# A-Nasiri-M/sap3d_tensorflow

Hardware: AMD Instinct MI355X
Metric: clips/s (16x112x112 fwd+bwd) (higher is better)
Workload: dtype f32

## Files before the change

### sap3d_tensorflow_amd/csrc/head.hip

```cpp
#include "p3d_kernels.h"
#include "det_reduce.h"

namespace {

__device__ __forceinline__ float4 ld4(const float* p) { return *reinterpret_cast<const float4*>(p); }

__global__ __launch_bounds__(256) void head_fwd_kernel(HeadArgs a) {
    P3D_CHAIN_PRIO();
    extern __shared__ float kw[];
    const int C = a.C;
    for (int i = threadIdx.x; i < 27 * C; i += blockDim.x) kw[i] = a.k[i];
    __syncthreads();
    const long long total = (long long)a.N * a.D * a.H * a.W;
    const float bias = a.bias[0];
    for (long long g = (long long)blockIdx.x * blockDim.x + threadIdx.x; g < total; g += (long long)gridDim.x * blockDim.x) {
        long long t = g;
        const int w = (int)(t % a.W); t /= a.W;
        const int h = (int)(t % a.H); t /= a.H;
        const int d = (int)(t % a.D); const int n = (int)(t / a.D);
        float out[8];
#pragma unroll
        for (int q = 0; q < 8; ++q) out[q] = bias;
        for (int dd = 0; dd < 2; ++dd) {
            if (d - dd < 0) continue;
            for (int dh = 0; dh < 2; ++dh) {
                if (h - dh < 0) continue;
                for (int dw = 0; dw < 2; ++dw) {
                    if (w - dw < 0) continue;
                    const float* xr = a.x + ((((long long)n * a.D + (d - dd)) * a.H + (h - dh)) * a.W + (w - dw)) * C;
                    const int nkd = dd ? 1 : 2, nkh = dh ? 1 : 2, nkw = dw ? 1 : 2;
                    for (int c = 0; c < C; c += 4) {
                        const float4 xv = ld4(xr + c);
                        for (int a0 = 0; a0 < nkd; ++a0) {
                            const int kd = dd ? 2 : a0, pd = dd ? 0 : a0;
                            for (int a1 = 0; a1 < nkh; ++a1) {
                                const int kh = dh ? 2 : a1, ph = dh ? 0 : a1;
                                for (int a2 = 0; a2 < nkw; ++a2) {
                                    const int kk = dw ? 2 : a2, pw = dw ? 0 : a2;
                                    const float* kp = kw + ((kd * 3 + kh) * 3 + kk) * C + c;
                                    out[(pd * 2 + ph) * 2 + pw] += xv.x * kp[0] + xv.y * kp[1] + xv.z * kp[2] + xv.w * kp[3];
                                }
                            }
                        }
                    }
                }
            }
        }
        const int Do = 2 * a.D, Ho = 2 * a.H, Wo = 2 * a.W;
#pragma unroll
        for (int pd = 0; pd < 2; ++pd)
#pragma unroll
            for (int ph = 0; ph < 2; ++ph) {
                const long long o = (((long long)n * Do + 2 * d + pd) * Ho + 2 * h + ph) * Wo + 2 * w;
                const float v0 = out[(pd * 2 + ph) * 2], v1 = out[(pd * 2 + ph) * 2 + 1];
                *reinterpret_cast<float2*>(a.logits + o) = make_float2(v0, v1);
                *reinterpret_cast<float2*>(a.pred + o) =
                    a.sigmoid ? make_float2(1.f / (1.f + expf(-v0)), 1.f / (1.f + expf(-v1))) : make_float2(v0, v1);
            }
    }
}

template <int L>
__global__ __launch_bounds__(256) void head_fwd_lanes_kernel(HeadArgs a) {
    P3D_CHAIN_PRIO();
    extern __shared__ float kw[];
    const int C = a.C;
    for (int i = threadIdx.x; i < 27 * C; i += blockDim.x) kw[i] = a.k[i];
    __syncthreads();
    const long long total = (long long)a.N * a.D * a.H * a.W;
    const float bias = a.bias[0];
    const int part = threadIdx.x % L, c = part * 4;
    const long long stride = (long long)gridDim.x * (256 / L);
    for (long long g = (long long)blockIdx.x * (256 / L) + threadIdx.x / L; g < total; g += stride) {
        long long t = g;
        const int w = (int)(t % a.W); t /= a.W;
        const int h = (int)(t % a.H); t /= a.H;
        const int d = (int)(t % a.D); const int n = (int)(t / a.D);
        float out[8];
#pragma unroll
        for (int q = 0; q < 8; ++q) out[q] = 0.f;
#pragma unroll
        for (int dd = 0; dd < 2; ++dd)
#pragma unroll
            for (int dh = 0; dh < 2; ++dh)
#pragma unroll
                for (int dw = 0; dw < 2; ++dw) {
                    if (d - dd < 0 || h - dh < 0 || w - dw < 0) continue;
                    const float4 xv = ld4(a.x + ((((long long)n * a.D + (d - dd)) * a.H + (h - dh)) * a.W + (w - dw)) * C + c);
#pragma unroll
                    for (int a0 = 0; a0 < (dd ? 1 : 2); ++a0)
#pragma unroll
                        for (int a1 = 0; a1 < (dh ? 1 : 2); ++a1)
#pragma unroll
                            for (int a2 = 0; a2 < (dw ? 1 : 2); ++a2) {
                                const int kd = dd ? 2 : a0, pd = dd ? 0 : a0, kh = dh ? 2 : a1, ph = dh ? 0 : a1, kk = dw ? 2 : a2, pw = dw ? 0 : a2;
                                const float4 kv = *reinterpret_cast<const float4*>(kw + ((kd * 3 + kh) * 3 + kk) * C + c);
                                out[(pd * 2 + ph) * 2 + pw] += xv.x * kv.x + xv.y * kv.y + xv.z * kv.z + xv.w * kv.w;
                            }
                }
#pragma unroll
        for (int o = L / 2; o > 0; o >>= 1)
#pragma unroll
            for (int q = 0; q < 8; ++q) out[q] += __shfl_xor(out[q], o);
        if (part == 0) {
            const int Do = 2 * a.D, Ho = 2 * a.H, Wo = 2 * a.W;
#pragma unroll
            for (int pd = 0; pd < 2; ++pd)
#pragma unroll
                for (int ph = 0; ph < 2; ++ph) {
                    const long long o = (((long long)n * Do + 2 * d + pd) * Ho + 2 * h + ph) * Wo + 2 * w;
                    const float v0 = out[(pd * 2 + ph) * 2] + bias, v1 = out[(pd * 2 + ph) * 2 + 1] + bias;
                    *reinterpret_cast<float2*>(a.logits + o) = make_float2(v0, v1);
                    *reinterpret_cast<float2*>(a.pred + o) =
                        a.sigmoid ? make_float2(1.f / (1.f + expf(-v0)), 1.f / (1.f + expf(-v1))) : make_float2(v0, v1);
                }
        }
    }
}

__global__ __launch_bounds__(256) void head_bwd_input_kernel(HeadArgs a) {
    P3D_CHAIN_PRIO();
    extern __shared__ float kw[];
    const int C = a.C, c4n = C >> 2;
    for (int i = threadIdx.x; i < 27 * C; i += blockDim.x) kw[i] = a.k[i];
    __syncthreads();
    const long long total = (long long)a.N * a.D * a.H * a.W * c4n;
    const int Do = 2 * a.D, Ho = 2 * a.H, Wo = 2 * a.W;
    for (long long i = (long long)blockIdx.x * blockDim.x + threadIdx.x; i < total; i += (long long)gridDim.x * blockDim.x) {
        long long t = i / c4n;
        const int c = (int)(i - t * c4n) << 2;
        const long long g = t;
        const int w = (int)(t % a.W); t /= a.W;
        const int h = (int)(t % a.H); t /= a.H;
        const int d = (int)(t % a.D); const int n = (int)(t / a.D);
        float4 acc = make_float4(0.f, 0.f, 0.f, 0.f);
        for (int kd = 0; kd < 3; ++kd) {
            const int od = 2 * d + kd;
            if (od >= Do) continue;
            for (int kh = 0; kh < 3; ++kh) {
                const int oh = 2 * h + kh;
                if (oh >= Ho) continue;
                for (int kk = 0; kk < 3; ++kk) {
                    const int ow = 2 * w + kk;
                    if (ow >= Wo) continue;
                    const float gdl = a.dlogits[(((long long)n * Do + od) * Ho + oh) * Wo + ow];
                    const float* kp = kw + ((kd * 3 + kh) * 3 + kk) * C + c;
                    acc.x += gdl * kp[0]; acc.y += gdl * kp[1]; acc.z += gdl * kp[2]; acc.w += gdl * kp[3];
                }
            }
        }
        *reinterpret_cast<float4*>(a.dx + g * C + c) = acc;
    }
}

__global__ __launch_bounds__(256) void head_bwd_filter_kernel(HeadArgs a) {
    __shared__ float red[256];
    const int C = a.C;
    const int lanes = 256 / C;
    const int c = threadIdx.x % C, sub = threadIdx.x / C;
    const long long total = (long long)a.N * a.D * a.H * a.W;
    const int Do = 2 * a.D, Ho = 2 * a.H, Wo = 2 * a.W;
    float acc[27];
#pragma unroll
    for (int q = 0; q < 27; ++q) acc[q] = 0.f;
    float bsum = 0.f;
    if (sub < lanes) {
        for (long long g = (long long)blockIdx.x * lanes + sub; g < total; g += (long long)gridDim.x * lanes) {
            long long t = g;
            const int w = (int)(t % a.W); t /= a.W;
            const int h = (int)(t % a.H); t /= a.H;
            const int d = (int)(t % a.D); const int n = (int)(t / a.D);
            const float xv = a.x[g * C + c];
#pragma unroll
            for (int kd = 0; kd < 3; ++kd)
#pragma unroll
                for (int kh = 0; kh < 3; ++kh)
#pragma unroll
                    for (int kk = 0; kk < 3; ++kk) {
                        const int od = 2 * d + kd, oh = 2 * h + kh, ow = 2 * w + kk;
                        float gdl = 0.f;
                        if (od < Do && oh < Ho && ow < Wo) gdl = a.dlogits[(((long long)n * Do + od) * Ho + oh) * Wo + ow];
                        acc[(kd * 3 + kh) * 3 + kk] += gdl * xv;
                        if (c == 0 && kd < 2 && kh < 2 && kk < 2) bsum += gdl;
                    }
        }
    }
    for (int q = 0; q < 27; ++q) {
        red[threadIdx.x] = (sub < lanes) ? acc[q] : 0.f;
        __syncthreads();
        if (threadIdx.x < C) {
            float s = 0.f;
            for (int l = 0; l < lanes; ++l) s += red[l * C + threadIdx.x];
            p3d_store_wt(a.part, ((size_t)blockIdx.x * 28 + q) * C + threadIdx.x, s);
        }
        __syncthreads();
    }
    red[threadIdx.x] = (sub < lanes && c == 0) ? bsum : 0.f;
    __syncthreads();
    if (threadIdx.x == 0) {
        float s = 0.f;
        for (int l = 0; l < lanes; ++l) s += red[l * C];
        p3d_store_wt(a.part, ((size_t)blockIdx.x * 28 + 27) * C, s);
    }
    __shared__ int last_flag;
    if (!p3d_last_block_wt(a.counter, gridDim.x, &last_flag)) return;
    for (int i = threadIdx.x; i < 27 * C + 1; i += blockDim.x) {
        const size_t slot = i < 27 * C ? (size_t)i : (size_t)27 * C;
        float t = 0.f;
#pragma unroll 8
        for (unsigned b = 0; b < gridDim.x; ++b) t += a.part[(size_t)b * 28 * C + slot];
        if (i < 27 * C) a.dk[i] += t; else a.dbias[0] += t;
    }
}

constexpr int HEAD_FOLD = 32;
__global__ __launch_bounds__(256) void head_bwd_filter4_kernel(HeadArgs a) {
    __shared__ float4 red[256];
    __shared__ int last_flag;
    const int C = a.C, L = C >> 2, R = 256 / L;
    const int lane = threadIdx.x % L, rs = threadIdx.x / L;
    const bool live = rs < R;
    const long long total = (long long)a.N * a.D * a.H * a.W;
    const int Do = 2 * a.D, Ho = 2 * a.H, Wo = 2 * a.W;
    float4 acc[27];
#pragma unroll
    for (int q = 0; q < 27; ++q) acc[q] = make_float4(0.f, 0.f, 0.f, 0.f);
    float bsum = 0.f;
    if (live) {
        for (long long g = (long long)blockIdx.x * R + rs; g < total; g += (long long)gridDim.x * R) {
            long long t = g;
            const int w = (int)(t % a.W); t /= a.W;
            const int h = (int)(t % a.H); t /= a.H;
            const int d = (int)(t % a.D); const int n = (int)(t / a.D);
            const float4 xv = *reinterpret_cast<const float4*>(a.x + g * C + lane * 4);
#pragma unroll
            for (int kd = 0; kd < 3; ++kd)
#pragma unroll
                for (int kh = 0; kh < 3; ++kh)
#pragma unroll
                    for (int kk = 0; kk < 3; ++kk) {
                        const int od = 2 * d + kd, oh = 2 * h + kh, ow = 2 * w + kk;
                        float gdl = 0.f;
                        if (od < Do && oh < Ho && ow < Wo) gdl = a.dlogits[(((long long)n * Do + od) * Ho + oh) * Wo + ow];
                        float4& s = acc[(kd * 3 + kh) * 3 + kk];
                        s.x = fmaf(gdl, xv.x, s.x); s.y = fmaf(gdl, xv.y, s.y); s.z = fmaf(gdl, xv.z, s.z); s.w = fmaf(gdl, xv.w, s.w);
                        if (lane == 0 && kd < 2 && kh < 2 && kk < 2) bsum += gdl;
                    }
        }
    }
#pragma unroll
    for (int q = 0; q < 27; ++q) {
        red[threadIdx.x] = live ? acc[q] : make_float4(0.f, 0.f, 0.f, 0.f);
        __syncthreads();
        if (threadIdx.x < L) {
            float4 s = red[threadIdx.x];
            for (int r = 1; r < R; ++r) { const float4 v = red[r * L + threadIdx.x]; s.x += v.x; s.y += v.y; s.z += v.z; s.w += v.w; }
            p3d_store_wt4(a.part, (size_t)blockIdx.x * 28 * C + q * C + threadIdx.x * 4, s);
        }
        __syncthreads();
    }
    red[threadIdx.x].x = (live && lane == 0) ? bsum : 0.f;
    __syncthreads();
    if (threadIdx.x == 0) {
        float s = 0.f;
        for (int r = 0; r < R; ++r) s += red[r * L].x;
        p3d_store_wt(a.part, (size_t)blockIdx.x * 28 * C + 27 * C, s);
    }
    const int nvals = 27 * C + 1;
    const unsigned ngroups = (gridDim.x + HEAD_FOLD - 1) / HEAD_FOLD, group = blockIdx.x / HEAD_FOLD;
    const unsigned first = group * HEAD_FOLD, in_group = min((unsigned)HEAD_FOLD, gridDim.x - first);
    float* gpart = a.part + (size_t)gridDim.x * 28 * C;
    if (!p3d_last_block_wt(a.counter + 1 + group, in_group, &last_flag)) return;
    for (int i = threadIdx.x; i < nvals; i += blockDim.x) {
        float t = 0.f;
#pragma unroll 8
        for (unsigned b = 0; b < in_group; ++b) t += a.part[(size_t)(first + b) * 28 * C + i];
        p3d_store_wt(gpart, (size_t)group * 28 * C + i, t);
    }
    if (!p3d_last_block_wt(a.counter, ngroups, &last_flag)) return;
    for (int i = threadIdx.x; i < nvals; i += blockDim.x) {
        float t = 0.f;
#pragma unroll 8
        for (unsigned gidx = 0; gidx < ngroups; ++gidx) t += gpart[(size_t)gidx * 28 * C + i];
        if (i < 27 * C) a.dk[i] += t; else a.dbias[0] += t;
    }
}

__global__ __launch_bounds__(256) void headc_fwd_kernel(HeadArgs a) {
    P3D_CHAIN_PRIO();
    extern __shared__ float kw[];
    const int C = a.C;
    for (int i = threadIdx.x; i < 27 * C; i += blockDim.x) kw[i] = a.k[i];
    __syncthreads();
    const long long total = (long long)a.N * a.D * a.H * a.W;
    const float bias = a.bias[0];
    for (long long g = (long long)blockIdx.x * blockDim.x + threadIdx.x; g < total; g += (long long)gridDim.x * blockDim.x) {
        long long t = g;
        const int w = (int)(t % a.W); t /= a.W;
        const int h = (int)(t % a.H); t /= a.H;
        const int d = (int)(t % a.D); const int n = (int)(t / a.D);
        float out = bias;
        for (int kd = 0; kd < 3; ++kd) {
            const int id = d + kd - 1;
            if (id < 0 || id >= a.D) continue;
            for (int kh = 0; kh < 3; ++kh) {
                const int ih = h + kh - 1;
                if (ih < 0 || ih >= a.H) continue;
                for (int kk = 0; kk < 3; ++kk) {
                    const int iw = w + kk - 1;
                    if (iw < 0 || iw >= a.W) continue;
                    const float* xr = a.x + ((((long long)n * a.D + id) * a.H + ih) * a.W + iw) * C;
                    const float* kp = kw + ((kd * 3 + kh) * 3 + kk) * C;
                    for (int c = 0; c < C; c += 4) {
                        const float4 xv = ld4(xr + c);
                        out += xv.x * kp[c] + xv.y * kp[c + 1] + xv.z * kp[c + 2] + xv.w * kp[c + 3];
                    }
                }
            }
        }
        a.logits[g] = out;
        a.pred[g] = a.sigmoid ? 1.f / (1.f + expf(-out)) : out;
    }
}

__global__ __launch_bounds__(256) void headc_bwd_input_kernel(HeadArgs a) {
    P3D_CHAIN_PRIO();
    extern __shared__ float kw[];
    const int C = a.C, c4n = C >> 2;
    for (int i = threadIdx.x; i < 27 * C; i += blockDim.x) kw[i] = a.k[i];
    __syncthreads();
    const long long total = (long long)a.N * a.D * a.H * a.W * c4n;
    for (long long i = (long long)blockIdx.x * blockDim.x + threadIdx.x; i < total; i += (long long)gridDim.x * blockDim.x) {
        long long t = i / c4n;
        const int c = (int)(i - t * c4n) << 2;
        const long long g = t;
        const int w = (int)(t % a.W); t /= a.W;
        const int h = (int)(t % a.H); t /= a.H;
        const int d = (int)(t % a.D); const int n = (int)(t / a.D);
        float4 acc = make_float4(0.f, 0.f, 0.f, 0.f);
        for (int kd = 0; kd < 3; ++kd) {
            const int od = d - kd + 1;
            if (od < 0 || od >= a.D) continue;
            for (int kh = 0; kh < 3; ++kh) {
                const int oh = h - kh + 1;
                if (oh < 0 || oh >= a.H) continue;
                for (int kk = 0; kk < 3; ++kk) {
                    const int ow = w - kk + 1;
                    if (ow < 0 || ow >= a.W) continue;
                    const float gdl = a.dlogits[(((long long)n * a.D + od) * a.H + oh) * a.W + ow];
                    const float* kp = kw + ((kd * 3 + kh) * 3 + kk) * C + c;
                    acc.x += gdl * kp[0]; acc.y += gdl * kp[1]; acc.z += gdl * kp[2]; acc.w += gdl * kp[3];
                }
            }
        }
        *reinterpret_cast<float4*>(a.dx + g * C + c) = acc;
    }
}

__global__ __launch_bounds__(256) void headc_bwd_filter_kernel(HeadArgs a) {
    __shared__ float red[256];
    const int C = a.C;
    const int lanes = 256 / C;
    const int c = threadIdx.x % C, sub = threadIdx.x / C;
    const long long total = (long long)a.N * a.D * a.H * a.W;
    float acc[27];
#pragma unroll
    for (int q = 0; q < 27; ++q) acc[q] = 0.f;
    float bsum = 0.f;
    if (sub < lanes) {
        for (long long g = (long long)blockIdx.x * lanes + sub; g < total; g += (long long)gridDim.x * lanes) {
            long long t = g;
            const int w = (int)(t % a.W); t /= a.W;
            const int h = (int)(t % a.H); t /= a.H;
            const int d = (int)(t % a.D); const int n = (int)(t / a.D);
            const float xv = a.x[g * C + c];
            if (c == 0) bsum += a.dlogits[g];
#pragma unroll
            for (int kd = 0; kd < 3; ++kd)
#pragma unroll
                for (int kh = 0; kh < 3; ++kh)
#pragma unroll
                    for (int kk = 0; kk < 3; ++kk) {
                        const int od = d - kd + 1, oh = h - kh + 1, ow = w - kk + 1;
                        float gdl = 0.f;
                        if (od >= 0 && od < a.D && oh >= 0 && oh < a.H && ow >= 0 && ow < a.W)
                            gdl = a.dlogits[(((long long)n * a.D + od) * a.H + oh) * a.W + ow];
                        acc[(kd * 3 + kh) * 3 + kk] += gdl * xv;
                    }
        }
    }
    for (int q = 0; q < 27; ++q) {
        red[threadIdx.x] = (sub < lanes) ? acc[q] : 0.f;
        __syncthreads();
        if (threadIdx.x < C) {
            float s = 0.f;
            for (int l = 0; l < lanes; ++l) s += red[l * C + threadIdx.x];
            p3d_store_wt(a.part, ((size_t)blockIdx.x * 28 + q) * C + threadIdx.x, s);
        }
        __syncthreads();
    }
    red[threadIdx.x] = (sub < lanes && c == 0) ? bsum : 0.f;
    __syncthreads();
    if (threadIdx.x == 0) {
        float s = 0.f;
        for (int l = 0; l < lanes; ++l) s += red[l * C];
        p3d_store_wt(a.part, ((size_t)blockIdx.x * 28 + 27) * C, s);
    }
    __shared__ int last_flag;
    if (!p3d_last_block_wt(a.counter, gridDim.x, &last_flag)) return;
    for (int i = threadIdx.x; i < 27 * C + 1; i += blockDim.x) {
        const size_t slot = i < 27 * C ? (size_t)i : (size_t)27 * C;
        float t = 0.f;
#pragma unroll 8
        for (unsigned b = 0; b < gridDim.x; ++b) t += a.part[(size_t)b * 28 * C + slot];
        if (i < 27 * C) a.dk[i] += t; else a.dbias[0] += t;
    }
}

}

hipError_t p3d_headc_fwd(const HeadArgs& a, hipStream_t s, HeadLaunch* done) {
    if ((a.C & 3) || a.C < 4 || a.C > 256) return hipErrorInvalidValue;
    const long long total = (long long)a.N * a.D * a.H * a.W;
    long long b = (total + 255) / 256;
    if (b > 8192) b = 8192;
    hipLaunchKernelGGL(headc_fwd_kernel, dim3((unsigned)b), dim3(256), 27 * a.C * sizeof(float), s, a);
    if (done) { done->kernel = P3D_HEAD_STRIDE1; done->blocks = (unsigned)b; }
    return hipGetLastError();
}

hipError_t p3d_headc_bwd_input(const HeadArgs& a, hipStream_t s) {
    if ((a.C & 3) || a.C < 4 || a.C > 256) return hipErrorInvalidValue;
    const long long total = (long long)a.N * a.D * a.H * a.W * (a.C >> 2);
    long long b = (total + 255) / 256;
    if (b > 8192) b = 8192;
    hipLaunchKernelGGL(headc_bwd_input_kernel, dim3((unsigned)b), dim3(256), 27 * a.C * sizeof(float), s, a);
    return hipGetLastError();
}

hipError_t p3d_headc_bwd_filter(const HeadArgs& a, hipStream_t s, HeadLaunch* done) {
    if (a.C > 256 || a.C < 1) return hipErrorInvalidValue;
    const long long total = (long long)a.N * a.D * a.H * a.W;
    const int lanes = 256 / a.C;
    long long b = (total + (long long)lanes * 32 - 1) / ((long long)lanes * 32);
    if (b > 256) b = 256;
    if (b < 1) b = 1;
    HeadArgs aa = a;
    const hipError_t e = p3d_stream_scratch(s, (size_t)b * 28 * a.C, 1, &aa.part, &aa.counter);
    if (e != hipSuccess) return e;
    hipLaunchKernelGGL(headc_bwd_filter_kernel, dim3((unsigned)b), dim3(256), 0, s, aa);
    if (done) { done->kernel = P3D_HEAD_STRIDE1; done->blocks = (unsigned)b; }
    return hipGetLastError();
}

hipError_t p3d_head_fwd(const HeadArgs& a, hipStream_t s, int path, HeadLaunch* done) {
    if ((a.C & 3) || a.C < 4 || a.C > 256) return hipErrorInvalidValue;
    if (path != P3D_HEAD_RULE && path != P3D_HEAD_LANES && path != P3D_HEAD_GENERIC) return hipErrorInvalidValue;
    const long long total = (long long)a.N * a.D * a.H * a.W;
    const int L = a.C >> 2;
    const bool lanes_ok = L > 1 && L <= 64 && (L & (L - 1)) == 0 && (reinterpret_cast<uintptr_t>(a.x) & 15) == 0;
    if (path == P3D_HEAD_LANES && !lanes_ok) return hipErrorInvalidValue;
    if (path == P3D_HEAD_LANES || (path == P3D_HEAD_RULE && lanes_ok)) {
        long long b = (total * L + 255) / 256;
        if (b > 16384) b = 16384;
        const size_t sm = 27 * a.C * sizeof(float);
#define P3D_HL(L_) case L_: hipLaunchKernelGGL(head_fwd_lanes_kernel<L_>, dim3((unsigned)b), dim3(256), sm, s, a); break;
        switch (L) { P3D_HL(2) P3D_HL(4) P3D_HL(8) P3D_HL(16) P3D_HL(32) P3D_HL(64) }
#undef P3D_HL
        if (done) { done->kernel = P3D_HEAD_LANES; done->blocks = (unsigned)b; }
        return hipGetLastError();
    }
    long long b = (total + 255) / 256;
    if (b > 8192) b = 8192;
    hipLaunchKernelGGL(head_fwd_kernel, dim3((unsigned)b), dim3(256), 27 * a.C * sizeof(float), s, a);
    if (done) { done->kernel = P3D_HEAD_GENERIC; done->blocks = (unsigned)b; }
    return hipGetLastError();
}

hipError_t p3d_head_bwd_input(const HeadArgs& a, hipStream_t s) {
    if ((a.C & 3) || a.C < 4 || a.C > 256) return hipErrorInvalidValue;
    const long long total = (long long)a.N * a.D * a.H * a.W * (a.C >> 2);
    long long b = (total + 255) / 256;
    if (b > 8192) b = 8192;
    hipLaunchKernelGGL(head_bwd_input_kernel, dim3((unsigned)b), dim3(256), 27 * a.C * sizeof(float), s, a);
    return hipGetLastError();
}

hipError_t p3d_head_bwd_filter(const HeadArgs& a, hipStream_t s, int path, HeadLaunch* done) {
    if (a.C > 256 || a.C < 1) return hipErrorInvalidValue;
    if (path != P3D_HEAD_RULE && path != P3D_HEAD_FILTER4 && path != P3D_HEAD_FILTER1) return hipErrorInvalidValue;
    const long long total = (long long)a.N * a.D * a.H * a.W;
    const bool four_ok = (a.C & 3) == 0 && (reinterpret_cast<uintptr_t>(a.x) & 15) == 0;
    if (path == P3D_HEAD_FILTER4 && !four_ok) return hipErrorInvalidValue;
    if (path == P3D_HEAD_FILTER4 || (path == P3D_HEAD_RULE && four_ok)) {
        const int R = 256 / (a.C >> 2);
        long long b = (total + (long long)R * 4 - 1) / ((long long)R * 4);
        if (b > 1024) b = 1024;
        if (b < 1) b = 1;
        const long long groups = (b + HEAD_FOLD - 1) / HEAD_FOLD;
        HeadArgs aa = a;
        const hipError_t e = p3d_stream_scratch(s, (size_t)(b + groups) * 28 * a.C, (int)(1 + groups), &aa.part, &aa.counter);
        if (e != hipSuccess) return e;
        hipLaunchKernelGGL(head_bwd_filter4_kernel, dim3((unsigned)b), dim3(256), 0, s, aa);
        if (done) { done->kernel = P3D_HEAD_FILTER4; done->blocks = (unsigned)b; }
        return hipGetLastError();
    }
    const int lanes = 256 / a.C;
    long long b = (total + (long long)lanes * 32 - 1) / ((long long)lanes * 32);
    if (b > 256) b = 256;
    if (b < 1) b = 1;
    HeadArgs aa = a;
    const hipError_t e = p3d_stream_scratch(s, (size_t)b * 28 * a.C, 1, &aa.part, &aa.counter);
    if (e != hipSuccess) return e;
    hipLaunchKernelGGL(head_bwd_filter_kernel, dim3((unsigned)b), dim3(256), 0, s, aa);
    if (done) { done->kernel = P3D_HEAD_FILTER1; done->blocks = (unsigned)b; }
    return hipGetLastError();
}
```

Measured before the change: 527.0.

## Keep head taps in registers, use DPP reductions and 32-bit indexing

For lane counts up to 16, the forward head kernel now loads its 27 filter taps per channel group into registers instead of staging them in shared memory. It issues all eight input loads up front, reduces across lanes with DPP row shifts, and caps the grid at a resident-sized launch. The input-gradient kernel is rebuilt the same way: one thread group per voxel, register-held taps, branch-free clamped loads, and 32-bit index math when the volume is small enough. The filter-gradient block reduction moves to wave-level DPP/shuffle sums followed by one cross-wave shared pass, replacing 27 barrier pairs. The cost is higher register pressure under a launch bound of 3 blocks per CU, and the DPP lane-above adds must line up correctly with the lane layout.

```diff
diff --git a/sap3d_tensorflow_amd/csrc/head.hip b/sap3d_tensorflow_amd/csrc/head.hip
--- a/sap3d_tensorflow_amd/csrc/head.hip
+++ b/sap3d_tensorflow_amd/csrc/head.hip
@@ -60,9 +60,108 @@
     }
 }
 
+__device__ __forceinline__ void head_position(const HeadArgs& a, long long g, bool narrow, int& n, int& d, int& h, int& w) {
+    if (narrow) {
+        unsigned t = (unsigned)g;
+        w = (int)(t % (unsigned)a.W); t /= (unsigned)a.W;
+        h = (int)(t % (unsigned)a.H); t /= (unsigned)a.H;
+        d = (int)(t % (unsigned)a.D); n = (int)(t / (unsigned)a.D);
+    } else {
+        long long t = g;
+        w = (int)(t % a.W); t /= a.W;
+        h = (int)(t % a.H); t /= a.H;
+        d = (int)(t % a.D); n = (int)(t / a.D);
+    }
+}
+
+template <int O>
+__device__ __forceinline__ float add_from_lane_above(float v) {
+    const int up = __builtin_amdgcn_update_dpp(0, __float_as_int(v), 0x100 + O, 0xf, 0xf, true);
+    return v + __int_as_float(up);
+}
+
+__device__ __forceinline__ void head_taps(const HeadArgs& a, int c, float4 (&kv)[27]) {
+#pragma unroll
+    for (int q = 0; q < 27; ++q) {
+        const float* kp = a.k + q * a.C + c;
+        kv[q] = make_float4(kp[0], kp[1], kp[2], kp[3]);
+    }
+}
+
 template <int L>
-__global__ __launch_bounds__(256) void head_fwd_lanes_kernel(HeadArgs a) {
-    P3D_CHAIN_PRIO();
+__device__ __forceinline__ void head_fwd_lanes_resident(const HeadArgs& a) {
+    const int C = a.C;
+    const long long total = (long long)a.N * a.D * a.H * a.W;
+    const bool narrow = total < (1ll << 31);
+    const float bias = a.bias[0];
+    const int part = threadIdx.x % L, c = part * 4;
+    float4 kv[27];
+    head_taps(a, c, kv);
+    const long long stride = (long long)gridDim.x * (256 / L);
+    for (long long g = (long long)blockIdx.x * (256 / L) + threadIdx.x / L; g < total; g += stride) {
+        int n, d, h, w;
+        head_position(a, g, narrow, n, d, h, w);
+        float4 xs[8];
+#pragma unroll
+        for (int dd = 0; dd < 2; ++dd)
+#pragma unroll
+            for (int dh = 0; dh < 2; ++dh)
+#pragma unroll
+                for (int dw = 0; dw < 2; ++dw) {
+                    const bool in = d - dd >= 0 && h - dh >= 0 && w - dw >= 0;
+                    const int id = max(d - dd, 0), ih = max(h - dh, 0), iw = max(w - dw, 0);
+                    const float4 xv = ld4(a.x + ((((long long)n * a.D + id) * a.H + ih) * a.W + iw) * C + c);
+                    xs[(dd * 2 + dh) * 2 + dw] = in ? xv : make_float4(0.f, 0.f, 0.f, 0.f);
+                }
+        float out[8];
+#pragma unroll
+        for (int q = 0; q < 8; ++q) out[q] = 0.f;
+#pragma unroll
+        for (int dd = 0; dd < 2; ++dd)
+#pragma unroll
+            for (int dh = 0; dh < 2; ++dh)
+#pragma unroll
+                for (int dw = 0; dw < 2; ++dw) {
+                    const float4 xv = xs[(dd * 2 + dh) * 2 + dw];
+#pragma unroll
+                    for (int a0 = 0; a0 < (dd ? 1 : 2); ++a0)
+#pragma unroll
+                        for (int a1 = 0; a1 < (dh ? 1 : 2); ++a1)
+#pragma unroll
+                            for (int a2 = 0; a2 < (dw ? 1 : 2); ++a2) {
+                                const int kd = dd ? 2 : a0, pd = dd ? 0 : a0, kh = dh ? 2 : a1, ph = dh ? 0 : a1, kk = dw ? 2 : a2, pw = dw ? 0 : a2;
+                                const float4 k4 = kv[(kd * 3 + kh) * 3 + kk];
+                                out[(pd * 2 + ph) * 2 + pw] += xv.x * k4.x + xv.y * k4.y + xv.z * k4.z + xv.w * k4.w;
+                            }
+                }
+#pragma unroll
+        for (int q = 0; q < 8; ++q) {
+            float v = out[q];
+            if (L > 32) v += __shfl_xor(v, 32);
+            if (L > 16) v += __shfl_xor(v, 16);
+            if (L > 8) v = add_from_lane_above<8>(v);
+            if (L > 4) v = add_from_lane_above<4>(v);
+            if (L > 2) v = add_from_lane_above<2>(v);
+            out[q] = add_from_lane_above<1>(v);
+        }
+        if (part == 0) {
+            const int Do = 2 * a.D, Ho = 2 * a.H, Wo = 2 * a.W;
+#pragma unroll
+            for (int pd = 0; pd < 2; ++pd)
+#pragma unroll
+                for (int ph = 0; ph < 2; ++ph) {
+                    const long long o = (((long long)n * Do + 2 * d + pd) * Ho + 2 * h + ph) * Wo + 2 * w;
+                    const float v0 = out[(pd * 2 + ph) * 2] + bias, v1 = out[(pd * 2 + ph) * 2 + 1] + bias;
+                    *reinterpret_cast<float2*>(a.logits + o) = make_float2(v0, v1);
+                    *reinterpret_cast<float2*>(a.pred + o) =
+                        a.sigmoid ? make_float2(1.f / (1.f + expf(-v0)), 1.f / (1.f + expf(-v1))) : make_float2(v0, v1);
+                }
+        }
+    }
+}
+
+template <int L>
+__device__ __forceinline__ void head_fwd_lanes_staged(const HeadArgs& a) {
     extern __shared__ float kw[];
     const int C = a.C;
     for (int i = threadIdx.x; i < 27 * C; i += blockDim.x) kw[i] = a.k[i];
@@ -118,36 +217,41 @@
     }
 }
 
-__global__ __launch_bounds__(256) void head_bwd_input_kernel(HeadArgs a) {
+template <int L>
+__global__ __launch_bounds__(256, 3) void head_fwd_lanes_kernel(HeadArgs a) {
     P3D_CHAIN_PRIO();
-    extern __shared__ float kw[];
-    const int C = a.C, c4n = C >> 2;
-    for (int i = threadIdx.x; i < 27 * C; i += blockDim.x) kw[i] = a.k[i];
-    __syncthreads();
-    const long long total = (long long)a.N * a.D * a.H * a.W * c4n;
+    if constexpr (L <= 16) head_fwd_lanes_resident<L>(a); else head_fwd_lanes_staged<L>(a);
+}
+
+__global__ __launch_bounds__(256, 3) void head_bwd_input_kernel(HeadArgs a) {
+    P3D_CHAIN_PRIO();
+    const int C = a.C, L = C >> 2, R = 256 / L;
+    const int part = threadIdx.x % L, rs = threadIdx.x / L, c = part * 4;
+    if (rs >= R) return;
+    const long long total = (long long)a.N * a.D * a.H * a.W;
+    const bool narrow = total < (1ll << 31);
     const int Do = 2 * a.D, Ho = 2 * a.H, Wo = 2 * a.W;
-    for (long long i = (long long)blockIdx.x * blockDim.x + threadIdx.x; i < total; i += (long long)gridDim.x * blockDim.x) {
-        long long t = i / c4n;
-        const int c = (int)(i - t * c4n) << 2;
-        const long long g = t;
-        const int w = (int)(t % a.W); t /= a.W;
-        const int h = (int)(t % a.H); t /= a.H;
-        const int d = (int)(t % a.D); const int n = (int)(t / a.D);
+    float4 kv[27];
+    head_taps(a, c, kv);
+    for (long long g = (long long)blockIdx.x * R + rs; g < total; g += (long long)gridDim.x * R) {
+        int n, d, h, w;
+        head_position(a, g, narrow, n, d, h, w);
+        float gdl[27];
+#pragma unroll
+        for (int kd = 0; kd < 3; ++kd)
+#pragma unroll
+            for (int kh = 0; kh < 3; ++kh)
+#pragma unroll
+                for (int kk = 0; kk < 3; ++kk) {
+                    const int od = 2 * d + kd, oh = 2 * h + kh, ow = 2 * w + kk;
+                    const bool in = od < Do && oh < Ho && ow < Wo;
+                    const float v = a.dlogits[(((long long)n * Do + min(od, Do - 1)) * Ho + min(oh, Ho - 1)) * Wo + min(ow, Wo - 1)];
+                    gdl[(kd * 3 + kh) * 3 + kk] = in ? v : 0.f;
+                }
         float4 acc = make_float4(0.f, 0.f, 0.f, 0.f);
-        for (int kd = 0; kd < 3; ++kd) {
-            const int od = 2 * d + kd;
-            if (od >= Do) continue;
-            for (int kh = 0; kh < 3; ++kh) {
-                const int oh = 2 * h + kh;
-                if (oh >= Ho) continue;
-                for (int kk = 0; kk < 3; ++kk) {
-                    const int ow = 2 * w + kk;
-                    if (ow >= Wo) continue;
-                    const float gdl = a.dlogits[(((long long)n * Do + od) * Ho + oh) * Wo + ow];
-                    const float* kp = kw + ((kd * 3 + kh) * 3 + kk) * C + c;
-                    acc.x += gdl * kp[0]; acc.y += gdl * kp[1]; acc.z += gdl * kp[2]; acc.w += gdl * kp[3];
-                }
-            }
+#pragma unroll
+        for (int q = 0; q < 27; ++q) {
+            acc.x += gdl[q] * kv[q].x; acc.y += gdl[q] * kv[q].y; acc.z += gdl[q] * kv[q].z; acc.w += gdl[q] * kv[q].w;
         }
         *reinterpret_cast<float4*>(a.dx + g * C + c) = acc;
     }
@@ -214,13 +318,51 @@
 }
 
 constexpr int HEAD_FOLD = 32;
+constexpr int HEAD_WAVE_RED = 4 * 27 * 16;
+
+template <int L>
+__device__ __forceinline__ float head_sum_wave_slots(float v) {
+    if (L <= 32) v += __shfl_down(v, 32);
+    if (L <= 16) v += __shfl_down(v, 16);
+    if (L <= 8) v = add_from_lane_above<8>(v);
+    if (L <= 4) v = add_from_lane_above<4>(v);
+    if (L <= 2) v = add_from_lane_above<2>(v);
+    if (L <= 1) v = add_from_lane_above<1>(v);
+    return v;
+}
+
+template <int L>
+__device__ __forceinline__ void head_filter4_block_sum(const HeadArgs& a, float4 (&acc)[27], float bsum, float4* red, float* bred) {
+    const int C = a.C, lane = threadIdx.x & 63, wave = threadIdx.x >> 6;
+#pragma unroll
+    for (int q = 0; q < 27; ++q) {
+        float4 s = acc[q];
+        s.x = head_sum_wave_slots<L>(s.x); s.y = head_sum_wave_slots<L>(s.y);
+        s.z = head_sum_wave_slots<L>(s.z); s.w = head_sum_wave_slots<L>(s.w);
+        if (lane < L) red[(wave * 27 + q) * L + lane] = s;
+    }
+    bsum = head_sum_wave_slots<L>(bsum);
+    if (lane == 0) bred[wave] = bsum;
+    __syncthreads();
+    for (int t = threadIdx.x; t < 27 * L; t += 256) {
+        const int q = t / L, l = t % L;
+        float4 s = red[q * L + l];
+#pragma unroll
+        for (int wv = 1; wv < 4; ++wv) { const float4 v = red[(wv * 27 + q) * L + l]; s.x += v.x; s.y += v.y; s.z += v.z; s.w += v.w; }
+        p3d_store_wt4(a.part, (size_t)blockIdx.x * 28 * C + q * C + l * 4, s);
+    }
+    if (threadIdx.x == 0) p3d_store_wt(a.part, (size_t)blockIdx.x * 28 * C + 27 * C, ((bred[0] + bred[1]) + bred[2]) + bred[3]);
+}
+
 __global__ __launch_bounds__(256) void head_bwd_filter4_kernel(HeadArgs a) {
-    __shared__ float4 red[256];
+    __shared__ float4 red[HEAD_WAVE_RED];
+    __shared__ float bred[4];
     __shared__ int last_flag;
     const int C = a.C, L = C >> 2, R = 256 / L;
     const int lane = threadIdx.x % L, rs = threadIdx.x / L;
     const bool live = rs < R;
     const long long total = (long long)a.N * a.D * a.H * a.W;
+    const bool narrow = total < (1ll << 31);
     const int Do = 2 * a.D, Ho = 2 * a.H, Wo = 2 * a.W;
     float4 acc[27];
 #pragma unroll
@@ -228,11 +370,10 @@
     float bsum = 0.f;
     if (live) {
         for (long long g = (long long)blockIdx.x * R + rs; g < total; g += (long long)gridDim.x * R) {
-            long long t = g;
-            const int w = (int)(t % a.W); t /= a.W;
-            const int h = (int)(t % a.H); t /= a.H;
-            const int d = (int)(t % a.D); const int n = (int)(t / a.D);
+            int n, d, h, w;
+            head_position(a, g, narrow, n, d, h, w);
             const float4 xv = *reinterpret_cast<const float4*>(a.x + g * C + lane * 4);
+            float gdl[27];
 #pragma unroll
             for (int kd = 0; kd < 3; ++kd)
 #pragma unroll
@@ -240,31 +381,48 @@
 #pragma unroll
                     for (int kk = 0; kk < 3; ++kk) {
                         const int od = 2 * d + kd, oh = 2 * h + kh, ow = 2 * w + kk;
-                        float gdl = 0.f;
-                        if (od < Do && oh < Ho && ow < Wo) gdl = a.dlogits[(((long long)n * Do + od) * Ho + oh) * Wo + ow];
+                        const bool in = od < Do && oh < Ho && ow < Wo;
+                        const float v = a.dlogits[(((long long)n * Do + min(od, Do - 1)) * Ho + min(oh, Ho - 1)) * Wo + min(ow, Wo - 1)];
+                        gdl[(kd * 3 + kh) * 3 + kk] = in ? v : 0.f;
+                    }
+#pragma unroll
+            for (int kd = 0; kd < 3; ++kd)
+#pragma unroll
+                for (int kh = 0; kh < 3; ++kh)
+#pragma unroll
+                    for (int kk = 0; kk < 3; ++kk) {
+                        const float t = gdl[(kd * 3 + kh) * 3 + kk];
                         float4& s = acc[(kd * 3 + kh) * 3 + kk];
-                        s.x = fmaf(gdl, xv.x, s.x); s.y = fmaf(gdl, xv.y, s.y); s.z = fmaf(gdl, xv.z, s.z); s.w = fmaf(gdl, xv.w, s.w);
-                        if (lane == 0 && kd < 2 && kh < 2 && kk < 2) bsum += gdl;
+                        s.x = fmaf(t, xv.x, s.x); s.y = fmaf(t, xv.y, s.y); s.z = fmaf(t, xv.z, s.z); s.w = fmaf(t, xv.w, s.w);
+                        if (lane == 0 && kd < 2 && kh < 2 && kk < 2) bsum += t;
                     }
         }
     }
-#pragma unroll
-    for (int q = 0; q < 27; ++q) {
-        red[threadIdx.x] = live ? acc[q] : make_float4(0.f, 0.f, 0.f, 0.f);
+    switch (L) {
+    case 1: head_filter4_block_sum<1>(a, acc, bsum, red, bred); break;
+    case 2: head_filter4_block_sum<2>(a, acc, bsum, red, bred); break;
+    case 4: head_filter4_block_sum<4>(a, acc, bsum, red, bred); break;
+    case 8: head_filter4_block_sum<8>(a, acc, bsum, red, bred); break;
+    case 16: head_filter4_block_sum<16>(a, acc, bsum, red, bred); break;
+    default:
+#pragma unroll
+        for (int q = 0; q < 27; ++q) {
+            red[threadIdx.x] = live ? acc[q] : make_float4(0.f, 0.f, 0.f, 0.f);
+            __syncthreads();
+            if (threadIdx.x < L) {
+                float4 s = red[threadIdx.x];
+                for (int r = 1; r < R; ++r) { const float4 v = red[r * L + threadIdx.x]; s.x += v.x; s.y += v.y; s.z += v.z; s.w += v.w; }
+                p3d_store_wt4(a.part, (size_t)blockIdx.x * 28 * C + q * C + threadIdx.x * 4, s);
+            }
+            __syncthreads();
+        }
+        red[threadIdx.x].x = (live && lane == 0) ? bsum : 0.f;
         __syncthreads();
-        if (threadIdx.x < L) {
-            float4 s = red[threadIdx.x];
-            for (int r = 1; r < R; ++r) { const float4 v = red[r * L + threadIdx.x]; s.x += v.x; s.y += v.y; s.z += v.z; s.w += v.w; }
-            p3d_store_wt4(a.part, (size_t)blockIdx.x * 28 * C + q * C + threadIdx.x * 4, s);
-        }
-        __syncthreads();
-    }
-    red[threadIdx.x].x = (live && lane == 0) ? bsum : 0.f;
-    __syncthreads();
-    if (threadIdx.x == 0) {
-        float s = 0.f;
-        for (int r = 0; r < R; ++r) s += red[r * L].x;
-        p3d_store_wt(a.part, (size_t)blockIdx.x * 28 * C + 27 * C, s);
+        if (threadIdx.x == 0) {
+            float s = 0.f;
+            for (int r = 0; r < R; ++r) s += red[r * L].x;
+            p3d_store_wt(a.part, (size_t)blockIdx.x * 28 * C + 27 * C, s);
+        }
     }
     const int nvals = 27 * C + 1;
     const unsigned ngroups = (gridDim.x + HEAD_FOLD - 1) / HEAD_FOLD, group = blockIdx.x / HEAD_FOLD;
@@ -419,6 +577,9 @@
 
 }
 
+constexpr long long HEAD_BLOCKS_PER_CU = 3;
+constexpr long long HEAD_RESIDENT = 256 * HEAD_BLOCKS_PER_CU;
+
 hipError_t p3d_headc_fwd(const HeadArgs& a, hipStream_t s, HeadLaunch* done) {
     if ((a.C & 3) || a.C < 4 || a.C > 256) return hipErrorInvalidValue;
     const long long total = (long long)a.N * a.D * a.H * a.W;
@@ -462,8 +623,9 @@
     if (path == P3D_HEAD_LANES && !lanes_ok) return hipErrorInvalidValue;
     if (path == P3D_HEAD_LANES || (path == P3D_HEAD_RULE && lanes_ok)) {
         long long b = (total * L + 255) / 256;
-        if (b > 16384) b = 16384;
-        const size_t sm = 27 * a.C * sizeof(float);
+        const long long cap = L <= 16 ? HEAD_RESIDENT : 16384;
+        if (b > cap) b = cap;
+        const size_t sm = L <= 16 ? 0 : 27 * a.C * sizeof(float);
 #define P3D_HL(L_) case L_: hipLaunchKernelGGL(head_fwd_lanes_kernel<L_>, dim3((unsigned)b), dim3(256), sm, s, a); break;
         switch (L) { P3D_HL(2) P3D_HL(4) P3D_HL(8) P3D_HL(16) P3D_HL(32) P3D_HL(64) }
 #undef P3D_HL
@@ -479,10 +641,11 @@
 
 hipError_t p3d_head_bwd_input(const HeadArgs& a, hipStream_t s) {
     if ((a.C & 3) || a.C < 4 || a.C > 256) return hipErrorInvalidValue;
-    const long long total = (long long)a.N * a.D * a.H * a.W * (a.C >> 2);
-    long long b = (total + 255) / 256;
-    if (b > 8192) b = 8192;
-    hipLaunchKernelGGL(head_bwd_input_kernel, dim3((unsigned)b), dim3(256), 27 * a.C * sizeof(float), s, a);
+    const long long total = (long long)a.N * a.D * a.H * a.W;
+    const int R = 256 / (a.C >> 2);
+    long long b = (total + R - 1) / R;
+    if (b > HEAD_RESIDENT) b = HEAD_RESIDENT;
+    hipLaunchKernelGGL(head_bwd_input_kernel, dim3((unsigned)b), dim3(256), 0, s, a);
     return hipGetLastError();
 }
 
```

Result: no change. 527.3 (median of 3 runs) (+0.1%).
